# wagnva/semantic-nerf-for-satellite-data

Measured on AMD Instinct MI355X. Metric: train rays/sec (4096 rays x 64 samples), higher is better.
Workload: dtype f32(f16x2)

## Files before the change

semantic-nerf-for-satellite-data_amd/csrc/api.hip:

```cpp
#include <stdarg.h>
#include <stdio.h>
#include <stdlib.h>
#include <string.h>

#include <mutex>

#include "aux_kernels.h"
#include "bsp.h"
#include "composite.h"
#include "gemm.h"
#include "plan.h"

namespace snerf {

int forward_bsp(const Plan& p, const float* pk, const SnerfInputs* in, const SnerfOutputs* out, void* workspace, hipStream_t st);
int backward_bsp(const Plan& p, const float* pk, const SnerfInputs* in, const SnerfOutGrads* go, float* gp, float* d_t, float* d_t_s,
                 void* workspace, hipStream_t st);

static thread_local char g_err[512] = "";
void set_error(const char* fmt, ...) {
  va_list ap;
  va_start(ap, fmt);
  vsnprintf(g_err, sizeof(g_err), fmt, ap);
  va_end(ap);
// ... 269 lines not shown
namespace {
struct BufNote { const void* p; bool composed; };
constexpr int NOTE_MAX = 256;
BufNote g_notes[NOTE_MAX];
int g_n_notes = 0, g_note_next = 0;
std::mutex g_note_mu;
void note_plan(const void* buf, bool composed) {
  std::lock_guard<std::mutex> lk(g_note_mu);
  for (int i = 0; i < g_n_notes; ++i) if (g_notes[i].p == buf) { g_notes[i].composed = composed; return; }
  if (g_n_notes < NOTE_MAX) g_notes[g_n_notes++] = {buf, composed};
  else { g_notes[g_note_next] = {buf, composed}; g_note_next = (g_note_next + 1) % NOTE_MAX; }
}
int check_plan_note(const void* buf, bool composed, const char* who, const char* what) {
  std::lock_guard<std::mutex> lk(g_note_mu);
  for (int i = 0; i < g_n_notes; ++i)
    if (g_notes[i].p == buf && g_notes[i].composed != composed) {
      set_error("%s: the %s was written under SNERF_COMPOSE_FEATS=%d, this call is planned with %d (pack, forward and backward must agree)",
                who, what, g_notes[i].composed ? 1 : 0, composed ? 1 : 0);
      return SNERF_ERR_BAD_DESC;
    }
  return SNERF_OK;
}
}

static int check_inputs(const Plan& p, const SnerfInputs* in) {
  if (!in) { set_error("null inputs"); return SNERF_ERR_NULL; }
  if (!in->sun_d || in->sun_stride < 3) { set_error("sun_d (N,3) with stride >= 3 is required"); return SNERF_ERR_NULL; }
  if (!in->t) { set_error("t (N,tau) is required"); return SNERF_ERR_NULL; }
  if (p.x_ts >= 0 && !in->t_s) { set_error("t_s is required with use_separate_tj_for_semantic"); return SNERF_ERR_NULL; }
  if (in->xyz) {
    if (!in->z_vals) { set_error("explicit xyz needs explicit z_vals"); return SNERF_ERR_NULL; }
  } else {
    if (!in->rays) { set_error("rays or xyz is required"); return SNERF_ERR_NULL; }
    if (!in->z_vals && !in->z_steps) { set_error("z_steps is required when z_vals is not given"); return SNERF_ERR_NULL; }
  }
  return SNERF_OK;
}

}

using namespace snerf;

extern "C" {

int snerf_version(void) { return SNERF_ABI_VERSION; }
const char* snerf_last_error(void) { return g_err; }

size_t snerf_packed_floats(const SnerfDesc* desc) {
  Plan p;
  if (make_plan(desc, &p)) return 0;
  return p.packed_floats;
}

size_t snerf_grad_floats(const SnerfDesc* desc) {
  Plan p;
  if (make_plan(desc, &p)) return 0;
  return p.n_fp32;
}

size_t snerf_workspace_bytes(const SnerfDesc* desc) {
  Plan p;
  if (make_plan(desc, &p)) return 0;
  return p.ws_bytes;
}

int snerf_pack_params(const SnerfDesc* desc, const SnerfParams* params, float* packed, void* stream) {
  Plan p;
  RC(make_plan(desc, &p));
  if (!params || !packed) { set_error("null params/packed"); return SNERF_ERR_NULL; }
  TableBuilder tb;
  build_tables(p, params, tb);
  if (tb.missing) { set_error("snerf_pack_params: a parameter tensor required by this SnerfDesc is NULL"); return SNERF_ERR_NULL; }
  hipStream_t st = (hipStream_t)stream;
  RC(launch_zero_bytes(packed, p.n_fp32 * sizeof(float), st));
  for (int i = 0; i < tb.nt; ++i) RC(launch_copy_table(tb.tabs[i], packed, 0, st));
  char* planes = reinterpret_cast<char*>(packed + p.n_fp32);
  int* exps = reinterpret_cast<int*>(planes + p.wp_bytes);
  unsigned* maxbits = reinterpret_cast<unsigned*>(exps + bsp::WPACK_MAX);
  note_plan(packed, p.compose_feats);
  if (!p.compose_feats) return bsp::launch_wpack(p.wj, packed, planes, exps, maxbits, p.pl, st);
  {
    bsp::SgTable tb;
    bsp::compose_jobs(tb, packed + p.w_h1, packed + p.w_fs, packed + p.b_fs, packed + p.b_h1, packed + p.o_wc, packed + p.o_bc, p.W, p.FA, p.N1);
    RC(bsp::launch_sgemm(tb, 64, st));
  }
  bsp::WPackTable first, rest;
  first.n = rest.n = 0;
  for (int i = 0; i < p.wj.n; ++i) (i < p.wj_first ? first.j[first.n++] : rest.j[rest.n++]) = p.wj.j[i];
  RC(bsp::launch_wpack(first, packed, planes, exps, maxbits, p.pl, st));
  return bsp::launch_wpack(rest, packed, planes, exps, maxbits, p.pl, st);
}

int snerf_unpack_grads(const SnerfDesc* desc, const float* packed_grads, const SnerfParams* grads, int accumulate,
                       void* stream) {
  Plan p;
  RC(make_plan(desc, &p));
  if (!grads || !packed_grads) { set_error("null grads"); return SNERF_ERR_NULL; }
  TableBuilder tb;
  build_tables(p, grads, tb);
  if (tb.missing) { set_error("snerf_unpack_grads: a gradient tensor required by this SnerfDesc is NULL"); return SNERF_ERR_NULL; }
  hipStream_t st = (hipStream_t)stream;
  for (int i = 0; i < tb.nt; ++i) RC(launch_copy_table(tb.tabs[i], const_cast<float*>(packed_grads), accumulate ? 2 : 1, st));
  return SNERF_OK;
}

int snerf_forward(const SnerfDesc* desc, const float* packed_params, const SnerfInputs* in, const SnerfOutputs* out,
                  void* workspace, size_t workspace_bytes, void* stream) {
  Plan p;
  RC(make_plan(desc, &p));
  if (!packed_params || !out || !workspace) { set_error("snerf_forward: null argument"); return SNERF_ERR_NULL; }
  if (workspace_bytes < p.ws_bytes) { set_error("snerf_forward: workspace too small (%zu < %zu)", workspace_bytes, p.ws_bytes); return SNERF_ERR_WORKSPACE; }
  if (((uintptr_t)workspace & 255) || ((uintptr_t)packed_params & 255)) { set_error("workspace and packed params must be 256-byte aligned"); return SNERF_ERR_WORKSPACE; }
  RC(check_inputs(p, in));
  RC(check_plan_note(packed_params, p.compose_feats, "snerf_forward", "packed parameter buffer"));
  note_plan(workspace, p.compose_feats);
  return forward_bsp(p, packed_params, in, out, workspace, (hipStream_t)stream);
}

int snerf_backward(const SnerfDesc* desc, const float* packed_params, const SnerfInputs* in, const SnerfOutGrads* gout,
                   float* packed_grads, float* d_t, float* d_t_s, void* workspace, size_t workspace_bytes, void* stream) {
  Plan p;
  RC(make_plan(desc, &p));
  if (!p.train) { set_error("snerf_backward needs the SnerfDesc used for the SNERF_FLAG_TRAIN forward"); return SNERF_ERR_BAD_DESC; }
  if (!packed_params || !gout || !packed_grads || !workspace) { set_error("snerf_backward: null argument"); return SNERF_ERR_NULL; }
  if (workspace_bytes < p.ws_bytes) { set_error("snerf_backward: workspace too small (%zu < %zu)", workspace_bytes, p.ws_bytes); return SNERF_ERR_WORKSPACE; }
  if (((uintptr_t)workspace & 255) || ((uintptr_t)packed_params & 255) || ((uintptr_t)packed_grads & 255)) { set_error("workspace and packed buffers must be 256-byte aligned"); return SNERF_ERR_WORKSPACE; }
  RC(check_inputs(p, in));
  RC(check_plan_note(packed_params, p.compose_feats, "snerf_backward", "packed parameter buffer"));
  RC(check_plan_note(workspace, p.compose_feats, "snerf_backward", "workspace"));
  return backward_bsp(p, packed_params, in, gout, packed_grads, d_t, d_t_s, workspace, (hipStream_t)stream);
}

int snerf_sample_z(const float* rays, const float* z_steps, const float* u, float* z, int n_rays, int n_samples, void* stream) {
  if (!rays || !z_steps || !z || n_rays <= 0 || n_samples <= 0) { set_error("snerf_sample_z: bad argument"); return SNERF_ERR_NULL; }
  return launch_sample_z(rays, z_steps, u, z, n_rays, n_samples, (hipStream_t)stream);
}

int snerf_embedding_rows(const float* table, int n_embed, int tau, const long long* idx, int n, float* rows, void* stream) {
  if (!table || !idx || !rows || n_embed <= 0 || tau <= 0 || n <= 0) { set_error("snerf_embedding_rows: bad argument"); return SNERF_ERR_NULL; }
  return launch_embedding_rows(table, n_embed, tau, idx, n, rows, (hipStream_t)stream);
}

int snerf_embedding_backward(const long long* idx, const float* d_rows, int n, int tau, int n_embed, float* grad_table, void* stream) {
  if (!idx || !d_rows || !grad_table || n_embed <= 0 || tau <= 0 || n <= 0) { set_error("snerf_embedding_backward: bad argument"); return SNERF_ERR_NULL; }
  return launch_embedding_backward(idx, d_rows, n, tau, n_embed, grad_table, (hipStream_t)stream);
}

int snerf_profile_begin(void) { return profile_begin(); }
int snerf_profile_end(SnerfProfile* out) { return profile_end(out); }

}
```

semantic-nerf-for-satellite-data_amd/csrc/bsp.h:

```cpp
#pragma once
#include "common.h"
#include "gemm.h"

namespace snerf {
namespace bsp {

constexpr int RB = 128;
constexpr int CB = 128;
constexpr int E_MAX = 100;
constexpr int E_QUIET = 60;

typedef __amdgpu_buffer_rsrc_t srd_t;
typedef unsigned int u32x4 __attribute__((ext_vector_type(4)));
typedef unsigned int u32x2 __attribute__((ext_vector_type(2)));
typedef _Float16 f16x8 __attribute__((ext_vector_type(8)));
typedef _Float16 f16x4 __attribute__((ext_vector_type(4)));
constexpr unsigned OOB = 0xFFFFFFF0u;

__host__ __device__ inline int ncb_of(int ld) { return (ld + CB - 1) / CB; }
__host__ __device__ inline size_t plane_bytes(size_t rows, int ld, int pl = 2) { return rows * (size_t)ld * 2 * pl; }
__host__ __device__ inline size_t etab_ints(size_t rows, int ld) { return ((rows + RB - 1) / RB) * (size_t)ncb_of(ld); }
__host__ __device__ inline unsigned g16_off(int k, int pl = 2) { return (unsigned)(k >> 4) * 32u * (unsigned)pl + (unsigned)(k & 15) * 2u; }

__host__ __device__ inline int exp_of_maxbits(unsigned b) {
// ... 81 lines not shown
  int rev = 0;
  int dbg = 0;
  int* tile_ctr = nullptr;
  int pl = 2;
  const float* nd_w = nullptr; float* nd_out = nullptr; unsigned long long nd_stride = 0;
  int nd_omax = 0, nd_ldw = 0;
  int nd_rows[8] = {0, 0, 0, 0, 0, 0, 0, 0}, nd_row0[8] = {0, 0, 0, 0, 0, 0, 0, 0}, nd_woff[8] = {0, 0, 0, 0, 0, 0, 0, 0};
};
__host__ __device__ inline size_t sign_words(size_t rows, int ld) { return ((rows + 31) / 32) * (size_t)((ld + 63) / 64) * 64; }

struct DwArgs {
  const char* A = nullptr; const int* EA = nullptr; int lda = 0; int a_col0 = 0;
  const char* B = nullptr; const int* EB = nullptr; int ldb = 0; int b_col0 = 0;
  int I = 0, J = 0, P = 0;
  float* C = nullptr; int ldc = 0;
  int k_split = 0, n_split = 1; unsigned long long slab_stride = 0;
  int tiles_i = 0, tiles_j = 0;
  int pl = 2;
};

constexpr int TR_MAXL = 8;
constexpr int TR_SLOTS = TR_MAXL + 1;
struct TrunkArgs {
  const char* pe = nullptr; const int* Epe = nullptr;
  int P = 0, W = 0, L = 0; unsigned skip_mask = 0;
  int gamma_free_layer = 0;
  const char* Wp[TR_SLOTS] = {}; const int* EW[TR_SLOTS] = {}; unsigned w_bytes[TR_SLOTS] = {}; int K[TR_SLOTS] = {};
  const float* bias[TR_SLOTS] = {}; float w0[TR_SLOTS] = {};
  char* F = nullptr; int* EF = nullptr; int ldf = 0;
  char* H[TR_MAXL] = {}; int* EH[TR_MAXL] = {}; unsigned* Hsign[TR_MAXL] = {};
  const float* nd_w = nullptr; float* nd_out = nullptr; unsigned long long nd_stride = 0;
  int* tile_ctr = nullptr;
  int dbg = 0;
};
inline int trunk_gamma_free_layer(int L, unsigned skip_mask) {
  int g = 2;
  for (int l = 2; l < L; ++l)
    if ((skip_mask >> l) & 1u) g = l;
  return g < L - 1 ? g : L - 1;
}
inline bool trunk_dma_in_final_layer(int L, unsigned skip_mask, bool feats_fused) {
  return !feats_fused && trunk_gamma_free_layer(L, skip_mask) == L - 1;
}
int launch_trunk(const TrunkArgs& a, bool train, hipStream_t st);
void trunk_set_grid_override(int n);
void trunk_set_fusion(int on);
bool trunk_fusion_enabled();

int launch_kc(const KcArgs& a, hipStream_t st);
void kc_set_grid_override(int n);
int launch_kc_narrow(const KcArgs& a, hipStream_t st);
int launch_dw(const DwArgs& a, bool narrow_i, hipStream_t st);

int launch_to_planes(const float* src, int ld_src, int rows, int cols, char* dst, int* E, int ld, int col0, int pl, hipStream_t st);
int launch_from_planes(const char* src, const int* E, int ld, int col0, int rows, int cols, float* dst, int ld_dst, int pl, hipStream_t st);

struct WPackJob {
  unsigned long long src_off;
  int src_ld;
  int rows, K;
  int transposed;
  unsigned long long dst_off;
  int e_idx;
  int m_rows, m_cols;
};
constexpr int WPACK_MAX = 48;
struct WPackTable { WPackJob j[WPACK_MAX]; int n; };
constexpr int WPACK_CHUNK = 24;
struct WPackChunk { WPackJob j[WPACK_CHUNK]; int n; };
__host__ __device__ inline size_t wp16_bytes(int rows, int K, int pl = 2) { return (size_t)((rows + 31) / 32) * (size_t)(K / 16) * 1024 * pl; }
int launch_wpack(const WPackTable& tb, const float* master, char* planes, int* exps, unsigned* maxbits, int pl, hipStream_t st);

struct SgJob {
  const float* A = nullptr; long long sa_i = 0, sa_k = 0;
  const float* B = nullptr; long long sb_k = 0, sb_j = 0;
  const float* D = nullptr; int ldd = 0;
  const float* u = nullptr; const float* v = nullptr;
  float* C = nullptr; int ldc = 0;
  int M = 0, N = 0, K = 0, acc = 0;
  int blk0 = 0;
};
constexpr int SG_MAX = 6;
struct SgTable { SgJob j[SG_MAX]; int n = 0; };
int launch_sgemm(const SgTable& tb, int tile_m, hipStream_t st);
void compose_jobs(SgTable& tb, const float* w_h1, const float* w_f, const float* b_f, const float* b_h1, float* wc, float* bc, int W, int FA, int N1);
void uncompose_jobs(SgTable& tb, const float* G, const float* gc, const float* w_h1, const float* w_f, const float* b_f,
                    float* dw_h1, float* db_h1, float* dw_f, float* db_f, int W, int FA, int M);

}
struct EncodeArgs;
namespace bsp {
int launch_encode_bsp(const EncodeArgs& a, char* pe, int* Epe, char* fa, int* Efa, int fa_col0, int pl, hipStream_t st);
int launch_zero_cols(char* base, size_t pitch, size_t width_bytes, int rows, hipStream_t st);
int launch_colsum32_bsp(const float* in, int rows, float* partial, char* planes, int* E, int pl, hipStream_t st);

}
}
```

semantic-nerf-for-satellite-data_amd/csrc/bsp_aux.hip:

```cpp
#include "bsp.h"
#include "aux_kernels.h"

namespace snerf {
namespace bsp {

__device__ __forceinline__ float block_max_256(float m, float* sm) {
#pragma unroll
  for (int o = 32; o >= 1; o >>= 1) m = fmaxf(m, __shfl_xor(m, o, 64));
  __syncthreads();
  if ((threadIdx.x & 63) == 0) sm[threadIdx.x >> 6] = m;
  __syncthreads();
  return fmaxf(fmaxf(sm[0], sm[1]), fmaxf(sm[2], sm[3]));
}

__global__ __launch_bounds__(256) void to_planes_kernel(const float* __restrict__ src, int ld_src, int rows, int cols,
                                                        char* __restrict__ dst, int* __restrict__ E, int ld, int col0, int pl) {
  __shared__ float sm[4];
  const int rb = blockIdx.y, cb = blockIdx.x;
  const int t = threadIdx.x, c8 = cb * 128 + (t & 15) * 8;
  float v[8][8];
  float m = 0.f;
#pragma unroll
  for (int i = 0; i < 8; ++i) {
    const int r = rb * 128 + (t >> 4) + 16 * i;
// ... 26 lines not shown
    set_error("to_planes: bad argument (ld % 16, col0 % 128)");
    return SNERF_ERR_BAD_DESC;
  }
  hipLaunchKernelGGL(to_planes_kernel, dim3((cols + 127) / 128, (rows + 127) / 128), dim3(256), 0, st, src, ld_src, rows, cols,
                     dst, E, ld, col0, pl);
  SNERF_LAUNCH_CHECK();
  return SNERF_OK;
}

__global__ void from_planes_kernel(const char* __restrict__ src, const int* __restrict__ E, int ld, int col0, int rows, int cols,
                                   float* __restrict__ dst, int ld_dst, int pl) {
  const size_t g = (size_t)blockIdx.x * blockDim.x + threadIdx.x;
  if (g >= (size_t)rows * cols) return;
  const int r = (int)(g / cols), c = (int)(g - (size_t)r * cols);
  const char* p = src + (size_t)r * ld * 2 * pl + g16_off(col0 + c, pl);
  const float hi = (float)*reinterpret_cast<const _Float16*>(p), lo = pl == 2 ? (float)*reinterpret_cast<const _Float16*>(p + 32) : 0.f;
  const int e = E[(size_t)(r >> 7) * ncb_of(ld) + ((col0 + c) >> 7)];
  dst[(size_t)r * ld_dst + c] = __builtin_amdgcn_ldexpf(hi + lo, -e);
}

int launch_from_planes(const char* src, const int* E, int ld, int col0, int rows, int cols, float* dst, int ld_dst, int pl, hipStream_t st) {
  const size_t n = (size_t)rows * cols;
  hipLaunchKernelGGL(from_planes_kernel, dim3((unsigned)((n + 255) / 256)), dim3(256), 0, st, src, E, ld, col0, rows, cols, dst, ld_dst, pl);
  SNERF_LAUNCH_CHECK();
  return SNERF_OK;
}

__global__ __launch_bounds__(256) void wmax_kernel(WPackChunk tb, const float* __restrict__ master, unsigned* __restrict__ maxbits) {
  const WPackJob j = tb.j[blockIdx.y];
  if (j.transposed == 1) return;
  float m = 0.f;
  const int wave = threadIdx.x >> 6, lane = threadIdx.x & 63;
  for (int r = blockIdx.x * 4 + wave; r < j.m_rows; r += gridDim.x * 4) {
    const float* row = master + j.src_off + (size_t)r * j.src_ld;
    for (int c = lane; c < j.m_cols; c += 64) m = fmaxf(m, fabsf(row[c]));
  }
#pragma unroll
  for (int o = 32; o >= 1; o >>= 1) m = fmaxf(m, __shfl_xor(m, o, 64));
  if ((threadIdx.x & 63) == 0 && m > 0.f) atomicMax(maxbits + j.e_idx, __float_as_uint(m));
}

__global__ __launch_bounds__(256) void wpack_kernel(WPackChunk tb, const float* __restrict__ master, char* __restrict__ planes,
                                                    int* __restrict__ exps, const unsigned* __restrict__ maxbits, int pl) {
  const WPackJob j = tb.j[blockIdx.y];
  const int rb32 = (j.rows + 31) >> 5, nks = j.K >> 4;
  const int e = exp_of_maxbits(maxbits[j.e_idx]);
  if (blockIdx.x == 0 && threadIdx.x == 0) exps[j.e_idx] = e;
  const float sc = pow2f(e);
  for (int unit = blockIdx.x; unit < rb32 * nks; unit += gridDim.x) {
    const int ks = unit / rb32, ub = unit - ks * rb32;
    const int r = threadIdx.x >> 3, kp = (threadIdx.x & 7) * 2;
    const int ra = ub * 32 + wf16_row(r), ka = ks * 16 + kp;
    float x[2];
#pragma unroll
    for (int q = 0; q < 2; ++q) {
      const int k = ka + q;
      const bool ok = j.transposed ? (k < j.m_rows && ra < j.m_cols) : (ra < j.m_rows && k < j.m_cols);
      x[q] = ok ? master[j.src_off + (j.transposed ? (size_t)k * j.src_ld + ra : (size_t)ra * j.src_ld + k)] : 0.f;
    }
    const _Float16 h0 = (_Float16)(x[0] * sc), h1 = (_Float16)(x[1] * sc);
    const _Float16 l0 = (_Float16)(x[0] * sc - (float)h0), l1 = (_Float16)(x[1] * sc - (float)h1);
    typedef _Float16 f16x2 __attribute__((ext_vector_type(2)));
    char* u = planes + j.dst_off + (size_t)unit * 1024 * pl + (32 * (kp >> 3) + r) * 16 + (kp & 7) * 2;
    *reinterpret_cast<f16x2*>(u) = f16x2{h0, h1};
    if (pl == 2) *reinterpret_cast<f16x2*>(u + 1024) = f16x2{l0, l1};
  }
}

int launch_wpack(const WPackTable& tb, const float* master, char* planes, int* exps, unsigned* maxbits, int pl, hipStream_t st) {
  if (tb.n <= 0) return SNERF_OK;
  { int rc = launch_zero_bytes(maxbits, WPACK_MAX * sizeof(unsigned), st); if (rc) return rc; }
  for (int pass = 0; pass < 2; ++pass)
    for (int first = 0; first < tb.n; first += WPACK_CHUNK) {
      WPackChunk c;
      c.n = tb.n - first < WPACK_CHUNK ? tb.n - first : WPACK_CHUNK;
      for (int i = 0; i < c.n; ++i) c.j[i] = tb.j[first + i];
      if (pass == 0) hipLaunchKernelGGL(wmax_kernel, dim3(32, c.n), dim3(256), 0, st, c, master, maxbits);
      else hipLaunchKernelGGL(wpack_kernel, dim3(128, c.n), dim3(256), 0, st, c, master, planes, exps, maxbits, pl);
      SNERF_LAUNCH_CHECK();
    }
  return SNERF_OK;
}

template <int TM>
__global__ __launch_bounds__(256) void sgemm_jobs_kernel(const SgTable tb) {
  constexpr int BM = 16 * TM, BN = 64, BK = 16;
  __shared__ float As[BK][BM + 1];
  __shared__ float Bs[BK][BN + 4];
  int q = 0;
  while (q + 1 < tb.n && (int)blockIdx.x >= tb.j[q + 1].blk0) ++q;
  const SgJob jb = tb.j[q];
  const int tiles_n = (jb.N + BN - 1) / BN;
  const int tile = (int)blockIdx.x - jb.blk0;
  const int i0 = (tile / tiles_n) * BM, j0 = (tile % tiles_n) * BN;
  const int t = threadIdx.x, ty = t >> 4, tx = t & 15;
  float acc[TM][4];
#pragma unroll
  for (int r = 0; r < TM; ++r)
#pragma unroll
    for (int c = 0; c < 4; ++c) acc[r][c] = 0.f;
  const bool a_k_fast = jb.sa_k == 1, b_j_fast = jb.sb_j == 1;
  for (int k0 = 0; k0 < jb.K; k0 += BK) {
#pragma unroll
    for (int s = 0; s < (BM * BK) / 256; ++s) {
      const int idx = t + 256 * s;
      const int i = a_k_fast ? idx / BK : idx % BM, k = a_k_fast ? idx % BK : idx / BM;
      As[k][i] = (i0 + i < jb.M && k0 + k < jb.K) ? jb.A[(long long)(i0 + i) * jb.sa_i + (long long)(k0 + k) * jb.sa_k] : 0.f;
    }
#pragma unroll
    for (int s = 0; s < (BN * BK) / 256; ++s) {
      const int idx = t + 256 * s;
      const int j = b_j_fast ? idx % BN : idx / BK, k = b_j_fast ? idx / BN : idx % BK;
      Bs[k][j] = (j0 + j < jb.N && k0 + k < jb.K) ? jb.B[(long long)(k0 + k) * jb.sb_k + (long long)(j0 + j) * jb.sb_j] : 0.f;
    }
    __syncthreads();
#pragma unroll
    for (int k = 0; k < BK; ++k) {
      float a[TM], b[4];
#pragma unroll
      for (int r = 0; r < TM; ++r) a[r] = As[k][ty * TM + r];
#pragma unroll
      for (int c = 0; c < 4; ++c) b[c] = Bs[k][tx * 4 + c];
#pragma unroll
      for (int r = 0; r < TM; ++r)
#pragma unroll
        for (int c = 0; c < 4; ++c) acc[r][c] = fmaf(a[r], b[c], acc[r][c]);
    }
    __syncthreads();
  }
#pragma unroll
  for (int r = 0; r < TM; ++r) {
    const int i = i0 + ty * TM + r;
    if (i >= jb.M) continue;
#pragma unroll
    for (int c = 0; c < 4; ++c) {
      const int j = j0 + tx * 4 + c;
      if (j >= jb.N) continue;
      float x = acc[r][c];
      if (jb.u) x = fmaf(jb.u[i], jb.v[j], x);
      if (jb.D) x += jb.D[(size_t)i * jb.ldd + j];
      float* o = jb.C + (size_t)i * jb.ldc + j;
      *o = jb.acc ? *o + x : x;
    }
  }
}

void compose_jobs(SgTable& tb, const float* w_h1, const float* w_f, const float* b_f, const float* b_h1, float* wc, float* bc, int W, int FA, int N1) {
  const int X = FA - W;
  tb.n = 0;
  auto job = [&]() -> SgJob& { tb.j[tb.n] = SgJob(); return tb.j[tb.n++]; };
  { SgJob& j = job(); j.A = w_h1; j.sa_i = FA; j.sa_k = 1; j.B = w_f; j.sb_k = W; j.sb_j = 1; j.C = wc; j.ldc = FA; j.M = N1; j.N = W; j.K = W; }
  { SgJob& j = job(); j.D = w_h1 + W; j.ldd = FA; j.C = wc + W; j.ldc = FA; j.M = N1; j.N = X; }
  { SgJob& j = job(); j.D = w_f + (size_t)W * W; j.ldd = W; j.C = wc + (size_t)N1 * FA; j.ldc = FA; j.M = 32; j.N = W; }
  { SgJob& j = job(); j.C = wc + (size_t)N1 * FA + W; j.ldc = FA; j.M = 32; j.N = X; }
  { SgJob& j = job(); j.A = w_h1; j.sa_i = FA; j.sa_k = 1; j.B = b_f; j.sb_k = 1; j.sb_j = 0; j.D = b_h1; j.ldd = 1; j.C = bc; j.ldc = 1; j.M = N1; j.N = 1; j.K = W; }
}
void uncompose_jobs(SgTable& tb, const float* G, const float* gc, const float* w_h1, const float* w_f, const float* b_f,
                    float* dw_h1, float* db_h1, float* dw_f, float* db_f, int W, int FA, int M) {
  tb.n = 0;
  auto job = [&]() -> SgJob& { tb.j[tb.n] = SgJob(); return tb.j[tb.n++]; };
  { SgJob& j = job(); j.A = G; j.sa_i = FA; j.sa_k = 1; j.B = w_f; j.sb_k = 1; j.sb_j = W; j.u = gc; j.v = b_f; j.C = dw_h1; j.ldc = FA; j.M = M; j.N = W; j.K = W; j.acc = 1; }
  { SgJob& j = job(); j.A = w_h1; j.sa_i = 1; j.sa_k = FA; j.B = G; j.sb_k = FA; j.sb_j = 1; j.C = dw_f; j.ldc = W; j.M = W; j.N = W; j.K = M; j.acc = 1; }
  { SgJob& j = job(); j.A = w_h1; j.sa_i = 1; j.sa_k = FA; j.B = gc; j.sb_k = 1; j.sb_j = 0; j.C = db_f; j.ldc = 1; j.M = W; j.N = 1; j.K = M; j.acc = 1; }
  { SgJob& j = job(); j.D = gc; j.ldd = 1; j.C = db_h1; j.ldc = 1; j.M = M; j.N = 1; j.acc = 1; }
}

int launch_sgemm(const SgTable& tb0, int tile_m, hipStream_t st) {
  if (tb0.n <= 0) return SNERF_OK;
  if (tb0.n > SG_MAX || (tile_m != 64 && tile_m != 32)) { set_error("sgemm: bad job table"); return SNERF_ERR_BAD_DESC; }
  SgTable tb = tb0;
  int blocks = 0;
  for (int q = 0; q < tb.n; ++q) {
    SgJob& j = tb.j[q];
    if (!j.C || j.M <= 0 || j.N <= 0 || j.K < 0 || j.ldc < 1 || (j.K > 0 && (!j.A || !j.B)) || (j.u && !j.v) || (j.D && j.ldd < 1)) {
      set_error("sgemm: bad job %d", q);
      return SNERF_ERR_BAD_DESC;
    }
    j.blk0 = blocks;
    blocks += ((j.M + tile_m - 1) / tile_m) * ((j.N + 63) / 64);
  }
  if (tile_m == 64) hipLaunchKernelGGL(sgemm_jobs_kernel<4>, dim3(blocks), dim3(256), 0, st, tb);
  else hipLaunchKernelGGL(sgemm_jobs_kernel<2>, dim3(blocks), dim3(256), 0, st, tb);
  SNERF_LAUNCH_CHECK();
  return SNERF_OK;
}

__global__ void zero_cols_kernel(char* base, size_t pitch, int width16, int rows) {
  const int i = blockIdx.x * blockDim.x + threadIdx.x;
  if (i >= rows * width16) return;
  const int r = i / width16, c = i - r * width16;
  *reinterpret_cast<u32x4*>(base + (size_t)r * pitch + 16 * (size_t)c) = u32x4{0u, 0u, 0u, 0u};
}
int launch_zero_cols(char* base, size_t pitch, size_t width_bytes, int rows, hipStream_t st) {
  const int w16 = (int)(width_bytes / 16);
  if (w16 <= 0 || rows <= 0) return SNERF_OK;
  hipLaunchKernelGGL(zero_cols_kernel, dim3((unsigned)(((size_t)rows * w16 + 255) / 256)), dim3(256), 0, st, base, pitch, w16, rows);
  SNERF_LAUNCH_CHECK();
  return SNERF_OK;
}

__device__ __forceinline__ void point_xyz(const EncodeArgs& a, long long point, float (&x)[3]) {
  const int n = (int)((unsigned)point / (unsigned)a.S);
#pragma unroll
  for (int c = 0; c < 3; ++c) {
    if (a.xyz != nullptr) {
      x[c] = a.xyz[point * 3 + c];
    } else {
#pragma clang fp contract(off)
      const float o = a.rays[n * 8 + c];
      const float d = a.dir_is_sun ? a.sun_d[(size_t)n * a.sun_stride + c] : a.rays[n * 8 + 3 + c];
      const float dz = d * a.z[point];
      x[c] = o + dz;
    }
  }
}
__device__ __forceinline__ float extras_value(const EncodeArgs& a, int n, int c) {
  if (c >= a.x_sun && c < a.x_sun + 3) return a.sun_d[(size_t)n * a.sun_stride + (c - a.x_sun)];
  if (a.t != nullptr && c >= a.x_t && c < a.x_t + a.tau) return a.t[(size_t)n * a.tau + (c - a.x_t)];
  if (a.t_s != nullptr && a.x_ts >= 0 && c >= a.x_ts && c < a.x_ts + a.tau) return a.t_s[(size_t)n * a.tau + (c - a.x_ts)];
  return 0.f;
}

struct EncodeBsp {
  EncodeArgs a;
  char* pe; int* Epe;
  char* fa; int* Efa; int fa_col0;
  int pl;
};

__global__ __launch_bounds__(256) void encode_bsp_kernel(EncodeBsp g) {
  __shared__ float sm[4];
  const EncodeArgs& a = g.a;
  const int rb = blockIdx.x, t = threadIdx.x;
  if (rb == 0) for (int i = t; i < a.zero_n; i += 256) a.zero[i] = 0u;
  const long long P = (long long)a.N * a.S;
  const long long p0 = (long long)rb * 128;
  const int npts = (int)min((long long)128, P - p0);
  float mx = 0.f, me = 0.f;
  if (a.F == 0)
    for (int i = t; i < npts; i += 256) {
      float x[3];
      point_xyz(a, p0 + i, x);
      mx = fmaxf(mx, fmaxf(fabsf(x[0]), fmaxf(fabsf(x[1]), fabsf(x[2]))));
    }
  if (g.fa != nullptr) {
    const int n0 = (int)((unsigned)p0 / (unsigned)a.S), n1 = (int)((unsigned)(p0 + npts - 1) / (unsigned)a.S);
    for (int i = t; i < (n1 - n0 + 1) * 16; i += 256) me = fmaxf(me, fabsf(extras_value(a, n0 + (i >> 4), i & 15)));
  }
  const int e_pe = a.F > 0 ? 13 : exp_of_maxbits(__float_as_uint(block_max_256(mx, sm)));
  const int e_x = g.fa != nullptr ? exp_of_maxbits(__float_as_uint(block_max_256(me, sm))) : 0;
  if (t == 0) {
    g.Epe[rb] = e_pe;
    if (g.fa != nullptr) g.Efa[(size_t)rb * ncb_of(a.FA) + (g.fa_col0 >> 7)] = e_x;
  }
  const float s_pe = pow2f(e_pe), s_x = pow2f(e_x);
  const int gpe = a.Ep >> 4, ngrp = gpe + (g.fa != nullptr ? 1 : 0);
  for (int item = t; item < npts * ngrp; item += 256) {
    const int pl = item / ngrp, grp = item - pl * ngrp;
    const long long point = p0 + pl;
    float v[16];
    char* d;
    float sc;
    if (grp < gpe) {
      float x[3];
      point_xyz(a, point, x);
// ... 118 lines not shown
```

semantic-nerf-for-satellite-data_amd/csrc/bsp_pass.hip:

```cpp
#include "aux_kernels.h"
#include "bsp.h"
#include "composite.h"
#include "plan.h"

namespace snerf {

namespace {
struct Ws {
  char* base;
  char* c(size_t off) const { return base + off; }
  float* f(size_t off) const { return reinterpret_cast<float*>(base + off); }
  int* i(size_t off) const { return reinterpret_cast<int*>(base + off); }
  unsigned* u(size_t off) const { return reinterpret_cast<unsigned*>(base + off); }
  void a(bsp::KcArgs& g, const PlaneT& t, int k, int col0 = 0) const { g.A = c(t.o); g.EA = i(t.e); g.lda = t.ld; g.a_col0 = col0; g.Ka = k; }
  void a2(bsp::KcArgs& g, const PlaneT& t) const { g.A2 = c(t.o); g.EA2 = i(t.e); g.lda2 = t.ld; }
  void out(bsp::KcArgs& g, const PlaneT& t, int col0 = 0) const { g.C = c(t.o); g.EC = i(t.e); g.ldc = t.ld; g.c_col0 = col0; g.Csign = t.s ? u(t.s) : nullptr; }
  void h(bsp::KcArgs& g, const PlaneT& t, int col0 = 0) const { g.H = c(t.o); g.EH = i(t.e); g.ldh = t.ld; g.h_col0 = col0; g.Hsign = t.s ? u(t.s) : nullptr; }
  void dz(bsp::DwArgs& g, const PlaneT& t) const { g.A = c(t.o); g.EA = i(t.e); g.lda = t.ld; g.a_col0 = 0; }
  void x(bsp::DwArgs& g, const PlaneT& t, int col0) const { g.B = c(t.o); g.EB = i(t.e); g.ldb = t.ld; g.b_col0 = col0; }
};
struct WOp { const char* W; const int* EW; int rb32; unsigned bytes; int K; };
WOp wop(const Plan& p, const float* pk, int job) {
  const char* planes = reinterpret_cast<const char*>(pk + p.n_fp32);
  const bsp::WPackJob& w = p.wj.j[job];
// ... 315 lines not shown
    const int r0 = p.sc ? p.sun_col : 0;
    const int nt = (P + 127) / 128, X = p.FA - W;
    RC(dw_gemm(r.w_h1, dz1, p.h1w, false, p.fa, 0, p.FA));
    RC(red_add_elem2d(rq.elem, r.w_h1.slab + W, r.w_h1.sp.ns, r.w_h1.stride, p.h1w, X, p.FA, gp + p.w_h1 + (size_t)r0 * p.FA + W, p.FA));
    RC(red_add_elem2d(rq.elem, r.w_h1.slab, r.w_h1.sp.ns, r.w_h1.stride, p.h1w, W, p.FA, r.w_h1.slab, p.FA));
    RC(red_store_last(rq.elem));
    RC(red_add_col(rq.col, r.cs_fin, nt, (size_t)r.ld_cs1, p.h1w, r.cs_fin));
    RC(red_store_last(rq.col));
    uncompose = true;
    RC(transient_grads());
    if (sig_live) {
      RC(narrow_grad(dsig, r.nar_sig, p.pdsig, gp + p.b_fs + W));
      RC(dw_gemm(r.w_fs, p.pdsig, NARROW, true, hl, 0, W));
      RC(dw_reduce(r.w_fs, (size_t)NARROW * W, gp + p.w_fs + (size_t)W * W));
    }
    { const PlaneT sw = dz_cur; dz_cur = dz_nxt; dz_nxt = sw; }
    bsp::KcArgs g;
    ws.a(g, dz1, p.h1w);
    if (sig_live) ws.a2(g, p.pdsig);
    weights(g, p, pk, p.wj_th1, 0, r0); g.I = P; g.J = W; g.K = sig_live ? p.h1w + NARROW : p.h1w;
    ws.out(g, dz_cur);
    dact(g, hl, 0, (p.L == 1) ? 30.f : 1.f);
    colsum(g, r.cs_hl, W);
    RC(launch_kc(g));
    RC(bias_from_colsum(r.cs_hl, W, gp + p.b_tr[p.L - 1]));
  }
  const PlaneT dfa = p.dzb.view(p.FA);
  if (!p.compose_feats) {
    const int r0 = p.sc ? p.sun_col : 0;
    RC(dw_gemm(r.w_h1, dz1, p.h1w, false, p.fa, 0, p.FA));
    RC(dw_reduce(r.w_h1, (size_t)p.h1w * p.FA, gp + p.w_h1 + (size_t)r0 * p.FA));
    bsp::KcArgs g;
    ws.a(g, dz1, p.h1w); weights(g, p, pk, p.wj_th1, 0, r0);
    g.I = P; g.J = W; g.K = p.h1w; ws.out(g, dfa);
    colsum(g, r.cs_fa, p.FA);
    RC(launch_kc(g));
    RC(red_add_col(rq.col, r.cs_fa, (P + 127) / 128, (size_t)cs_ld(p.FA), W, gp + p.b_fs));
    RC(transient_grads());
  }
  if (!p.compose_feats) {
    if (sig_live) RC(narrow_grad(dsig, r.nar_sig, p.pdsig, gp + p.b_fs + W));
    RC(dw_gemm(r.w_fs, dfa, W, false, hl, 0, W));
    if (sig_live) RC(dw_gemm(r.w_fs, p.pdsig, NARROW, true, hl, 0, W, (size_t)W * W));
    RC(dw_reduce(r.w_fs, (size_t)(sig_live ? W + NARROW : W) * W, gp + p.w_fs));
    bsp::KcArgs g;
    ws.a(g, dfa, W);
    if (sig_live) ws.a2(g, p.pdsig);
    weights(g, p, pk, p.wj_tfs); g.I = P; g.J = W; g.K = sig_live ? W + NARROW : W;
    ws.out(g, dz_cur);
    dact(g, hl, 0, (p.L == 1) ? 30.f : 1.f);
    colsum(g, r.cs_hl, W);
    RC(launch_kc(g));
    RC(bias_from_colsum(r.cs_hl, W, gp + p.b_tr[p.L - 1]));
  }
  for (int i = p.L - 1; i >= 0; --i) {
    const BwdRegions::Layer& t = r.tr[i];
    if (i > 0 && ((p.skip_mask >> i) & 1u)) {
      RC(dw_gemm(t.w_gamma, dz_cur, W, false, p.pe, 0, p.Ep));
      RC(dw_gemm(t.w, dz_cur, W, false, p.h[i - 1], 0, W));
      RC(red_add_elem2d(rq.elem, t.w_gamma.slab, t.w_gamma.sp.ns, t.w_gamma.stride, W, p.Ep, p.Ep, gp + p.w_tr[i], p.k_tr[i]));
      RC(red_add_elem2d(rq.elem, t.w.slab, t.w.sp.ns, t.w.stride, W, W, W, gp + p.w_tr[i] + p.Ep, p.k_tr[i]));
    } else {
      if (i == 0) RC(dw_gemm(t.w, dz_cur, W, false, p.pe, 0, p.Ep));
      else RC(dw_gemm(t.w, dz_cur, W, false, p.h[i - 1], 0, W));
      RC(dw_reduce(t.w, (size_t)W * p.k_tr[i], gp + p.w_tr[i]));
    }
    if (i == 0) break;
    bsp::KcArgs g;
    ws.a(g, dz_cur, W); weights(g, p, pk, p.wj_tt[i]);
    g.I = P; g.J = W; g.K = W; ws.out(g, dz_nxt);
    dact(g, p.h[i - 1], 0, (i - 1 == 0) ? 30.f : 1.f);
    colsum(g, t.cs, W);
    RC(launch_kc(g));
    RC(bias_from_colsum(t.cs, W, gp + p.b_tr[i - 1]));
    const PlaneT sw = dz_cur; dz_cur = dz_nxt; dz_nxt = sw;
  }
  RC(launch_reductions(rq.elem, rq.col, st));
  if (!uncompose) return SNERF_OK;
  {
    const size_t r0 = p.sc ? (size_t)p.sun_col : 0;
    bsp::SgTable tb;
    bsp::uncompose_jobs(tb, r.w_h1.slab, r.cs_fin, pk + p.w_h1 + r0 * p.FA, pk + p.w_fs, pk + p.b_fs,
                        gp + p.w_h1 + r0 * p.FA, gp + p.b_h1 + r0, gp + p.w_fs, gp + p.b_fs, W, p.FA, p.h1w);
    return bsp::launch_sgemm(tb, 32, st);
  }
}

}
```

Baseline: 170,700.

## Rewrite small fp32 job-table sgemm with register-prefetched vector loads and smaller tiles

Replaces the templated 256-thread sgemm used for weight compose/uncompose with a 128-thread, 64x32x32 tile kernel. Global loads become float4 where the stride and alignment allow, and the next K-slab is prefetched into registers while the current one is computed. Jobs are sorted by K so the longest blocks launch first. The aim is more blocks and better load efficiency for these small GEMMs, at the cost of more code paths and a unified tile size for both call sites.

```diff
diff --git a/semantic-nerf-for-satellite-data_amd/csrc/api.hip b/semantic-nerf-for-satellite-data_amd/csrc/api.hip
--- a/semantic-nerf-for-satellite-data_amd/csrc/api.hip
+++ b/semantic-nerf-for-satellite-data_amd/csrc/api.hip
@@ -375,7 +375,7 @@
   {
     bsp::SgTable tb;
     bsp::compose_jobs(tb, packed + p.w_h1, packed + p.w_fs, packed + p.b_fs, packed + p.b_h1, packed + p.o_wc, packed + p.o_bc, p.W, p.FA, p.N1);
-    RC(bsp::launch_sgemm(tb, 64, st));
+    RC(bsp::launch_sgemm(tb, st));
   }
   bsp::WPackTable first, rest;
   first.n = rest.n = 0;
diff --git a/semantic-nerf-for-satellite-data_amd/csrc/bsp.h b/semantic-nerf-for-satellite-data_amd/csrc/bsp.h
--- a/semantic-nerf-for-satellite-data_amd/csrc/bsp.h
+++ b/semantic-nerf-for-satellite-data_amd/csrc/bsp.h
@@ -187,7 +187,7 @@
 };
 constexpr int SG_MAX = 6;
 struct SgTable { SgJob j[SG_MAX]; int n = 0; };
-int launch_sgemm(const SgTable& tb, int tile_m, hipStream_t st);
+int launch_sgemm(const SgTable& tb, hipStream_t st);
 void compose_jobs(SgTable& tb, const float* w_h1, const float* w_f, const float* b_f, const float* b_h1, float* wc, float* bc, int W, int FA, int N1);
 void uncompose_jobs(SgTable& tb, const float* G, const float* gc, const float* w_h1, const float* w_f, const float* b_f,
                     float* dw_h1, float* db_h1, float* dw_f, float* db_f, int W, int FA, int M);
diff --git a/semantic-nerf-for-satellite-data_amd/csrc/bsp_aux.hip b/semantic-nerf-for-satellite-data_amd/csrc/bsp_aux.hip
--- a/semantic-nerf-for-satellite-data_amd/csrc/bsp_aux.hip
+++ b/semantic-nerf-for-satellite-data_amd/csrc/bsp_aux.hip
@@ -132,55 +132,107 @@
   return SNERF_OK;
 }
 
-template <int TM>
-__global__ __launch_bounds__(256) void sgemm_jobs_kernel(const SgTable tb) {
-  constexpr int BM = 16 * TM, BN = 64, BK = 16;
-  __shared__ float As[BK][BM + 1];
-  __shared__ float Bs[BK][BN + 4];
+namespace {
+constexpr int SG_BM = 64, SG_BN = 32, SG_BK = 32, SG_NT = 128;
+constexpr int SG_LDA = SG_BM + 4, SG_LDB = SG_BN + 4;
+
+__device__ __forceinline__ float4 sg_load4(const float* __restrict__ base, long long sf, long long ss, int f0, int nf, int s, int ns, bool vec) {
+  if (s >= ns) return make_float4(0.f, 0.f, 0.f, 0.f);
+  const float* p = base + (long long)s * ss;
+  if (vec && f0 + 3 < nf) return *reinterpret_cast<const float4*>(p + f0);
+  float v[4];
+#pragma unroll
+  for (int e = 0; e < 4; ++e) v[e] = f0 + e < nf ? p[(long long)(f0 + e) * sf] : 0.f;
+  return make_float4(v[0], v[1], v[2], v[3]);
+}
+__device__ __forceinline__ bool sg_vec_ok(const float* base, long long sf, long long ss) {
+  return sf == 1 && (ss & 3) == 0 && (reinterpret_cast<unsigned long long>(base) & 15ull) == 0;
+}
+}
+
+__global__ __launch_bounds__(SG_NT) void sgemm_jobs_kernel(const SgTable tb) {
+  constexpr int BM = SG_BM, BN = SG_BN, BK = SG_BK;
+  constexpr int NA = (BM * BK) / (4 * SG_NT), NB = (BN * BK) / (4 * SG_NT);
+  __shared__ __attribute__((aligned(16))) float As[BK][SG_LDA];
+  __shared__ __attribute__((aligned(16))) float Bs[BK][SG_LDB];
   int q = 0;
   while (q + 1 < tb.n && (int)blockIdx.x >= tb.j[q + 1].blk0) ++q;
   const SgJob jb = tb.j[q];
   const int tiles_n = (jb.N + BN - 1) / BN;
   const int tile = (int)blockIdx.x - jb.blk0;
   const int i0 = (tile / tiles_n) * BM, j0 = (tile % tiles_n) * BN;
-  const int t = threadIdx.x, ty = t >> 4, tx = t & 15;
-  float acc[TM][4];
-#pragma unroll
-  for (int r = 0; r < TM; ++r)
+  const int t = threadIdx.x, ty = t >> 3, tx = t & 7;
+  float acc[4][4];
+#pragma unroll
+  for (int r = 0; r < 4; ++r)
 #pragma unroll
     for (int c = 0; c < 4; ++c) acc[r][c] = 0.f;
   const bool a_k_fast = jb.sa_k == 1, b_j_fast = jb.sb_j == 1;
+  const long long a_sf = a_k_fast ? jb.sa_k : jb.sa_i, a_ss = a_k_fast ? jb.sa_i : jb.sa_k;
+  const long long b_sf = b_j_fast ? jb.sb_j : jb.sb_k, b_ss = b_j_fast ? jb.sb_k : jb.sb_j;
+  const bool a_vec = jb.K > 0 && sg_vec_ok(jb.A, a_sf, a_ss), b_vec = jb.K > 0 && sg_vec_ok(jb.B, b_sf, b_ss);
+  float4 ra[NA], rb[NB];
+  auto fetch = [&](int k0) {
+#pragma unroll
+    for (int s = 0; s < NA; ++s) {
+      const int idx = t + SG_NT * s;
+      ra[s] = a_k_fast ? sg_load4(jb.A, a_sf, a_ss, k0 + 4 * (idx & 7), jb.K, i0 + (idx >> 3), jb.M, a_vec)
+                       : sg_load4(jb.A, a_sf, a_ss, i0 + 4 * (idx & 15), jb.M, k0 + (idx >> 4), jb.K, a_vec);
+    }
+#pragma unroll
+    for (int s = 0; s < NB; ++s) {
+      const int idx = t + SG_NT * s;
+      rb[s] = b_j_fast ? sg_load4(jb.B, b_sf, b_ss, j0 + 4 * (idx & 7), jb.N, k0 + (idx >> 3), jb.K, b_vec)
+                       : sg_load4(jb.B, b_sf, b_ss, k0 + 4 * (idx & 7), jb.K, j0 + (idx >> 3), jb.N, b_vec);
+    }
+  };
+  auto stage = [&]() {
+#pragma unroll
+    for (int s = 0; s < NA; ++s) {
+      const int idx = t + SG_NT * s;
+      if (a_k_fast) {
+        const int k = 4 * (idx & 7), i = idx >> 3;
+        As[k][i] = ra[s].x; As[k + 1][i] = ra[s].y; As[k + 2][i] = ra[s].z; As[k + 3][i] = ra[s].w;
+      } else {
+        *reinterpret_cast<float4*>(&As[idx >> 4][4 * (idx & 15)]) = ra[s];
+      }
+    }
+#pragma unroll
+    for (int s = 0; s < NB; ++s) {
+      const int idx = t + SG_NT * s;
+      if (b_j_fast) {
+        *reinterpret_cast<float4*>(&Bs[idx >> 3][4 * (idx & 7)]) = rb[s];
+      } else {
+        const int k = 4 * (idx & 7), j = idx >> 3;
+        Bs[k][j] = rb[s].x; Bs[k + 1][j] = rb[s].y; Bs[k + 2][j] = rb[s].z; Bs[k + 3][j] = rb[s].w;
+      }
+    }
+  };
+  auto fma16 = [&](int k) {
+    const float4 a4 = *reinterpret_cast<const float4*>(&As[k][4 * ty]), b4 = *reinterpret_cast<const float4*>(&Bs[k][4 * tx]);
+    const float a[4] = {a4.x, a4.y, a4.z, a4.w}, b[4] = {b4.x, b4.y, b4.z, b4.w};
+#pragma unroll
+    for (int r = 0; r < 4; ++r)
+#pragma unroll
+      for (int c = 0; c < 4; ++c) acc[r][c] = fmaf(a[r], b[c], acc[r][c]);
+  };
+  if (jb.K > 0) fetch(0);
   for (int k0 = 0; k0 < jb.K; k0 += BK) {
-#pragma unroll
-    for (int s = 0; s < (BM * BK) / 256; ++s) {
-      const int idx = t + 256 * s;
-      const int i = a_k_fast ? idx / BK : idx % BM, k = a_k_fast ? idx % BK : idx / BM;
-      As[k][i] = (i0 + i < jb.M && k0 + k < jb.K) ? jb.A[(long long)(i0 + i) * jb.sa_i + (long long)(k0 + k) * jb.sa_k] : 0.f;
-    }
-#pragma unroll
-    for (int s = 0; s < (BN * BK) / 256; ++s) {
-      const int idx = t + 256 * s;
-      const int j = b_j_fast ? idx % BN : idx / BK, k = b_j_fast ? idx / BN : idx % BK;
-      Bs[k][j] = (j0 + j < jb.N && k0 + k < jb.K) ? jb.B[(long long)(k0 + k) * jb.sb_k + (long long)(j0 + j) * jb.sb_j] : 0.f;
-    }
+    stage();
     __syncthreads();
-#pragma unroll
-    for (int k = 0; k < BK; ++k) {
-      float a[TM], b[4];
-#pragma unroll
-      for (int r = 0; r < TM; ++r) a[r] = As[k][ty * TM + r];
-#pragma unroll
-      for (int c = 0; c < 4; ++c) b[c] = Bs[k][tx * 4 + c];
-#pragma unroll
-      for (int r = 0; r < TM; ++r)
-#pragma unroll
-        for (int c = 0; c < 4; ++c) acc[r][c] = fmaf(a[r], b[c], acc[r][c]);
+    if (k0 + BK < jb.K) fetch(k0 + BK);
+    if (jb.K - k0 > 16) {
+#pragma unroll
+      for (int k = 0; k < BK; ++k) fma16(k);
+    } else {
+#pragma unroll
+      for (int k = 0; k < 16; ++k) fma16(k);
     }
     __syncthreads();
   }
 #pragma unroll
-  for (int r = 0; r < TM; ++r) {
-    const int i = i0 + ty * TM + r;
+  for (int r = 0; r < 4; ++r) {
+    const int i = i0 + ty * 4 + r;
     if (i >= jb.M) continue;
 #pragma unroll
     for (int c = 0; c < 4; ++c) {
@@ -215,22 +267,26 @@
   { SgJob& j = job(); j.D = gc; j.ldd = 1; j.C = db_h1; j.ldc = 1; j.M = M; j.N = 1; j.acc = 1; }
 }
 
-int launch_sgemm(const SgTable& tb0, int tile_m, hipStream_t st) {
+int launch_sgemm(const SgTable& tb0, hipStream_t st) {
   if (tb0.n <= 0) return SNERF_OK;
-  if (tb0.n > SG_MAX || (tile_m != 64 && tile_m != 32)) { set_error("sgemm: bad job table"); return SNERF_ERR_BAD_DESC; }
+  if (tb0.n > SG_MAX) { set_error("sgemm: bad job table"); return SNERF_ERR_BAD_DESC; }
   SgTable tb = tb0;
+  for (int q = 0; q < tb.n; ++q) {
+    const SgJob& j = tb.j[q];
+    if (!j.C || j.M <= 0 || j.N <= 0 || j.K < 0 || j.ldc < 1 || (j.K > 0 && (!j.A || !j.B)) || (j.u && !j.v) || (j.D && j.ldd < 1)) {
+      set_error("sgemm: bad job %d", q);
+      return SNERF_ERR_BAD_DESC;
+    }
+  }
+  for (int q = 1; q < tb.n; ++q)
+    for (int r = q; r > 0 && tb.j[r].K > tb.j[r - 1].K; --r) { const SgJob s = tb.j[r]; tb.j[r] = tb.j[r - 1]; tb.j[r - 1] = s; }
   int blocks = 0;
   for (int q = 0; q < tb.n; ++q) {
     SgJob& j = tb.j[q];
-    if (!j.C || j.M <= 0 || j.N <= 0 || j.K < 0 || j.ldc < 1 || (j.K > 0 && (!j.A || !j.B)) || (j.u && !j.v) || (j.D && j.ldd < 1)) {
-      set_error("sgemm: bad job %d", q);
-      return SNERF_ERR_BAD_DESC;
-    }
     j.blk0 = blocks;
-    blocks += ((j.M + tile_m - 1) / tile_m) * ((j.N + 63) / 64);
-  }
-  if (tile_m == 64) hipLaunchKernelGGL(sgemm_jobs_kernel<4>, dim3(blocks), dim3(256), 0, st, tb);
-  else hipLaunchKernelGGL(sgemm_jobs_kernel<2>, dim3(blocks), dim3(256), 0, st, tb);
+    blocks += ((j.M + SG_BM - 1) / SG_BM) * ((j.N + SG_BN - 1) / SG_BN);
+  }
+  hipLaunchKernelGGL(sgemm_jobs_kernel, dim3(blocks), dim3(SG_NT), 0, st, tb);
   SNERF_LAUNCH_CHECK();
   return SNERF_OK;
 }
diff --git a/semantic-nerf-for-satellite-data_amd/csrc/bsp_pass.hip b/semantic-nerf-for-satellite-data_amd/csrc/bsp_pass.hip
--- a/semantic-nerf-for-satellite-data_amd/csrc/bsp_pass.hip
+++ b/semantic-nerf-for-satellite-data_amd/csrc/bsp_pass.hip
@@ -421,8 +421,8 @@
     bsp::SgTable tb;
     bsp::uncompose_jobs(tb, r.w_h1.slab, r.cs_fin, pk + p.w_h1 + r0 * p.FA, pk + p.w_fs, pk + p.b_fs,
                         gp + p.w_h1 + r0 * p.FA, gp + p.b_h1 + r0, gp + p.w_fs, gp + p.b_fs, W, p.FA, p.h1w);
-    return bsp::launch_sgemm(tb, 32, st);
-  }
-}
-
-}
+    return bsp::launch_sgemm(tb, st);
+  }
+}
+
+}
```

Result: no change. 171,600 (median of 6 runs) (+0.5%).
